# fegemo/palette-and-histo-gan

Hardware: AMD Instinct MI355X
Metric: train images/sec (64x64x4 sprites) (higher is better)
Workload: dtype bf16

## Files before the change

### palette_and_histo_gan_amd/csrc/conv_strip.hip

```cpp
#include "p2p_common.hpp"

struct CsArgs {
    const char* in; long long in_img; int in_row; int in_ld;
    char* out; long long out_img; int out_row; int out_ld;
    const char* w;
    float* stat_part;
    int LH, LW, lgLW;
    int TH, strips_per_img, nstrips;
    int RH, RW, PB;
    float inv_RW;
};

#define CS_MAXC 7
#define CS_THREADS 512

template <int MODE>
__global__ __launch_bounds__(CS_THREADS) void conv_strip_kernel(CsArgs a) {
    constexpr int NTAP = MODE == 1 ? 4 : 16;
    constexpr int KS = MODE == 1 ? 8 : 2;
    constexpr int CIN = KS * 16;
    constexpr int LGCPP = MODE == 1 ? 4 : 2;
    constexpr int PROW = 64 + 16;
    extern __shared__ __attribute__((aligned(16))) char smem[];
    const int tid = threadIdx.x, lane = tid & 63;
    const int wave = __builtin_amdgcn_readfirstlane(tid >> 6);
    const int h = lane >> 5, r = lane & 31;
    const int RW = a.RW, PB = a.PB;
    char* sL = smem;
    char* pL = smem + ((a.RH * RW * PB + 15) & ~15) + wave * (32 * PROW);
    const int slice = wave & 3, tpar = wave >> 2;
    const int ph = slice >> 1, pw = slice & 1;

    bf16x8 wf[NTAP][KS];
#pragma unroll
    for (int t = 0; t < NTAP; ++t) {
        int widx, row;
        if (MODE == 1) { widx = ((1 - ph) + 2 * (t >> 1)) * 4 + (1 - pw) + 2 * (t & 1); row = r; }
        else { widx = t; row = 32 * slice + r; }
        const int rows = MODE == 1 ? 32 : 128;
        const char* wp = a.w + ((long long)(widx * rows + row) * CIN) * 2;
#pragma unroll
        for (int ks = 0; ks < KS; ++ks) wf[t][ks] = *(const bf16x8*)(wp + (16 * ks + 8 * h) * 2);
    }

    const int nch = (a.RH * RW) << LGCPP;
    const int gpB = a.in_ld * 2;
    f32x4 stg[CS_MAXC];
    auto g_load = [&](int strip) {
        const int n = strip / a.strips_per_img, y0 = (strip - n * a.strips_per_img) * a.TH;
        const int oy = MODE == 1 ? y0 - 1 : 2 * y0 - 1;
        const char* base = a.in + ((long long)n * a.in_img + (long long)oy * a.in_row - 1) * gpB;
#pragma unroll
        for (int i = 0; i < CS_MAXC; ++i) {
            const int ci = tid + i * CS_THREADS;
            if (ci < nch) {
                const int px = ci >> LGCPP, cc = ci & ((1 << LGCPP) - 1);
                const int ry = (int)(((float)px + 0.5f) * a.inv_RW), rx = px - ry * RW;
                stg[i] = *(const f32x4*)(base + ((long long)ry * a.in_row + rx) * gpB + cc * 16);
            }
        }
    };
    auto l_store = [&]() {
#pragma unroll
        for (int i = 0; i < CS_MAXC; ++i) {
            const int ci = tid + i * CS_THREADS;
            if (ci < nch) *(f32x4*)(sL + (ci >> LGCPP) * PB + (ci & ((1 << LGCPP) - 1)) * 16) = stg[i];
        }
    };

    const int tiles = (a.TH * a.LW) >> 5;
    float* stL = (float*)(smem + ((a.RH * RW * PB + 15) & ~15) + 8 * (32 * PROW));
    int pend_n = -1, pend_s = 0;
    auto flush_stats = [&]() {
        if (tid < 32) {
            float s1 = 0.f, s2 = 0.f;
#pragma unroll
            for (int wv = 0; wv < 8; ++wv) { s1 += stL[(wv * 32 + tid) * 2]; s2 += stL[(wv * 32 + tid) * 2 + 1]; }
            const float cnt = (float)(4 * a.TH * a.LW);
            const float mean = s1 / cnt;
            float* dst = a.stat_part + (((long long)pend_n * a.strips_per_img + pend_s) * 32 + tid) * 2;
            dst[0] = mean;
            dst[1] = fmaxf(s2 - s1 * mean, 0.f);
        }
    };
    int strip = blockIdx.x;
    if (strip < a.nstrips) g_load(strip);
    for (; strip < a.nstrips; strip += gridDim.x) {
        __syncthreads();
        if (MODE == 1 && a.stat_part && pend_n >= 0) flush_stats();
        l_store();
        __syncthreads();
        if (strip + (int)gridDim.x < a.nstrips) g_load(strip + gridDim.x);
        const int n = strip / a.strips_per_img, sidx = strip - n * a.strips_per_img, y0 = sidx * a.TH;
        float ssum = 0.f, ssq = 0.f;
        for (int tile = tpar; tile < tiles; tile += 2) {
            const int p = tile * 32 + r;
            const int yy = p >> a.lgLW, x = p & (a.LW - 1);
            f32x16 acc;
            const float zero = p2p_valu_zero();
#pragma unroll
            for (int e = 0; e < 16; ++e) acc[e] = zero;
#pragma unroll
            for (int t = 0; t < NTAP; ++t) {
                int ry, rx;
                if (MODE == 1) {
                    const int kh = (1 - ph) + 2 * (t >> 1), kw = (1 - pw) + 2 * (t & 1);
                    ry = yy + 1 + ((ph + 1 - kh) >> 1);
                    rx = x + 1 + ((pw + 1 - kw) >> 1);
                } else { ry = 2 * yy + (t >> 2); rx = 2 * x + (t & 3); }
                const char* bp = sL + (ry * RW + rx) * PB + 16 * h;
#pragma unroll
                for (int ks = 0; ks < KS; ++ks) {
                    const bf16x8 b = *(const bf16x8*)(bp + 32 * ks);
                    acc = __builtin_amdgcn_mfma_f32_32x32x16_bf16(wf[t][ks], b, acc, 0, 0, 0);
                }
            }
#pragma unroll
            for (int g = 0; g < 4; ++g) {
                typedef __attribute__((__vector_size__(4 * sizeof(bf16_t)))) bf16_t bf16x4;
                bf16x4 q;
#pragma unroll
                for (int k = 0; k < 4; ++k) q[k] = (bf16_t)acc[4 * g + k];
                *(bf16x4*)(pL + r * PROW + (8 * g + 4 * h) * 2) = q;
            }
            asm volatile("s_waitcnt lgkmcnt(0)" ::: "memory");
            __builtin_amdgcn_wave_barrier();
            if (MODE == 1 && a.stat_part) {
                const bf16_t* col = (const bf16_t*)(pL + (16 * h) * PROW) + r;
#pragma unroll
                for (int i = 0; i < 16; ++i) {
                    const float v = (float)col[i * (PROW / 2)];
                    ssum += v;
                    ssq += v * v;
                }
            }
            const int ch = lane & 3, pq = lane >> 2;
#pragma unroll
            for (int ps = 0; ps < 32; ps += 16) {
                const int pix = ps + pq;
                const int pp = tile * 32 + pix;
                const int py = pp >> a.lgLW, px = pp & (a.LW - 1);
                const f32x4 v = *(const f32x4*)(pL + pix * PROW + ch * 16);
                long long opix;
                int c0;
                if (MODE == 1) { opix = (long long)n * a.out_img + (long long)(2 * (y0 + py) + ph) * a.out_row + (2 * px + pw); c0 = ch * 8; }
                else { opix = (long long)n * a.out_img + (long long)(y0 + py) * a.out_row + px; c0 = 32 * slice + ch * 8; }
                *(f32x4*)((bf16_t*)a.out + opix * a.out_ld + c0) = v;
            }
            __builtin_amdgcn_wave_barrier();
        }
        if (MODE == 1 && a.stat_part) {
            ssum += __shfl_xor(ssum, 32, 64);
            ssq += __shfl_xor(ssq, 32, 64);
            if (h == 0) { stL[(wave * 32 + r) * 2] = ssum; stL[(wave * 32 + r) * 2 + 1] = ssq; }
            pend_n = n; pend_s = sidx;
        }
    }
    if (MODE == 1 && a.stat_part && pend_n >= 0) {
        __syncthreads();
        flush_stats();
    }
}

struct CsPlan { int ok, TH, RH, RW, PB, blocks; size_t shm; };

static CsPlan cs_plan(int op, int dtype, int N, int LH, int LW, int Cg, int Cd) {
    CsPlan p = {0, 0, 0, 0, 0, 0, 0};
    if (dtype != P2P_BF16 || Cg != 32 || Cd != 128 || N < 1) return p;
    if (op != P2P_OP_G && op != P2P_OP_P) return p;
    if ((LW & (LW - 1)) || LW < 32 || LW > 128 || LH < 1) return p;
    const int cin = op == P2P_OP_P ? 128 : 32;
    p.PB = cin * 2 + 16;
    int TH = 0;
    for (int pass = 0; pass < 2 && !TH; ++pass)
        for (int t = 4; t >= (pass ? 1 : 2); t >>= 1) {
            if (t > LH || LH % t) continue;
            p.RH = op == P2P_OP_P ? t + 2 : 2 * t + 3;
            p.RW = op == P2P_OP_P ? LW + 2 : 2 * LW + 3;
            p.shm = (((size_t)p.RH * p.RW * p.PB + 15) & ~(size_t)15) + 8 * 32 * (size_t)(64 + 16) + 8 * 32 * 2 * sizeof(float);
            const long long nch = (long long)p.RH * p.RW * (cin / 8);
            if (nch > CS_MAXC * CS_THREADS) continue;
            if (((t * LW) >> 5) & 1) continue;
            if (p.shm <= (size_t)(pass ? 150 : 80) * 1024) { TH = t; break; }
        }
    if (!TH) return p;
    p.TH = TH;
    const long long strips = (long long)N * (LH / TH);
    if (strips > 0x7fffffffLL) return p;
    p.blocks = (int)(strips < 256 ? strips : 256);
    p.ok = 1;
    return p;
}

extern "C" int p2p_conv_strip_ok(int op, int dtype, int N, int LH, int LW, int Cg, int Cd) {
    return cs_plan(op, dtype, N, LH, LW, Cg, Cd).ok;
}

extern "C" int p2p_conv_strip_stat_slots(int op, int dtype, int N, int LH, int LW, int Cg, int Cd) {
    const CsPlan p = cs_plan(op, dtype, N, LH, LW, Cg, Cd);
    return (p.ok && op == P2P_OP_P) ? LH / p.TH : 0;
}

extern "C" int p2p_conv_strip(int op, int dtype, int N, int LH, int LW, int Cg, int Cd, const p2p_tensor* hi,
                              const p2p_tensor* lo, const void* w, float* stat_part, void* stream) {
    P2P_REQUIRE(hi && lo && hi->ptr && lo->ptr && w, "p2p_conv_strip: null pointer");
    const CsPlan p = cs_plan(op, dtype, N, LH, LW, Cg, Cd);
    P2P_REQUIRE(p.ok, "p2p_conv_strip: shape not supported (query p2p_conv_strip_ok)");
    const p2p_tensor* in = op == P2P_OP_G ? hi : lo;
    const p2p_tensor* out = op == P2P_OP_G ? lo : hi;
    const int cin = op == P2P_OP_P ? 128 : 32, cout = op == P2P_OP_P ? 32 : 128;
    P2P_REQUIRE(in->ld >= cin && in->ld % 8 == 0 && ((uintptr_t)in->ptr % 16) == 0 && ((uintptr_t)w % 16) == 0,
                "p2p_conv_strip: input view / weights must be 16-byte aligned");
    P2P_REQUIRE(out->ld >= cout && out->ld % 8 == 0 && ((uintptr_t)out->ptr % 16) == 0, "p2p_conv_strip: output view must be 16-byte aligned");
    CsArgs a;
    a.in = (const char*)in->ptr; a.in_img = in->img_stride; a.in_row = in->row_stride; a.in_ld = in->ld;
    a.out = (char*)out->ptr; a.out_img = out->img_stride; a.out_row = out->row_stride; a.out_ld = out->ld;
    a.w = (const char*)w;
    a.LH = LH; a.LW = LW;
    a.lgLW = 0;
    while ((1 << a.lgLW) < LW) ++a.lgLW;
    a.TH = p.TH; a.strips_per_img = LH / p.TH; a.nstrips = N * a.strips_per_img;
    a.RH = p.RH; a.RW = p.RW; a.PB = p.PB;
    a.inv_RW = 1.0f / (float)p.RW;
    a.stat_part = op == P2P_OP_P ? stat_part : nullptr;
    hipStream_t st = (hipStream_t)stream;
    const dim3 grid((unsigned)p.blocks);
    static bool attr_done = false;
    if (!attr_done)
        attr_done = (int)p2p_allow_lds((const void*)conv_strip_kernel<0>, 160 * 1024, "conv_strip_kernel<0>") &
                    (int)p2p_allow_lds((const void*)conv_strip_kernel<1>, 160 * 1024, "conv_strip_kernel<1>");
    if (op == P2P_OP_P) conv_strip_kernel<1><<<grid, dim3(CS_THREADS), p.shm, st>>>(a);
    else conv_strip_kernel<0><<<grid, dim3(CS_THREADS), p.shm, st>>>(a);
    return p2p_check_launch("p2p_conv_strip");
}
```

Baseline: 135,000.

## Carry halo rows between consecutive strips via LDS ring buffer

Switches from grid-strided strip assignment to contiguous strip ranges per block. Consecutive strips of the same image now reuse the two overlapping halo rows kept in an LDS ring buffer, so only the new rows are loaded from global memory. Tile x indexing is also simplified so each tile covers 32 pixels within one row. This adds ring-index arithmetic to the inner loop's address computation and relies on the assumption that a tile never straddles rows.

Result: no change. 136,300 (median of 6 runs) (+1.0%).

```diff
diff --git a/palette_and_histo_gan_amd/csrc/conv_strip.hip b/palette_and_histo_gan_amd/csrc/conv_strip.hip
--- a/palette_and_histo_gan_amd/csrc/conv_strip.hip
+++ b/palette_and_histo_gan_amd/csrc/conv_strip.hip
@@ -8,11 +8,16 @@
     int LH, LW, lgLW;
     int TH, strips_per_img, nstrips;
     int RH, RW, PB;
+    int RG;
     float inv_RW;
 };
 
 #define CS_MAXC 7
 #define CS_THREADS 512
+#define CS_KEEP 2
+#ifndef CS_CARRY_ROWS
+#define CS_CARRY_ROWS 1
+#endif
 
 template <int MODE>
 __global__ __launch_bounds__(CS_THREADS) void conv_strip_kernel(CsArgs a) {
@@ -25,7 +30,8 @@
     const int tid = threadIdx.x, lane = tid & 63;
     const int wave = __builtin_amdgcn_readfirstlane(tid >> 6);
     const int h = lane >> 5, r = lane & 31;
-    const int RW = a.RW, PB = a.PB;
+    const int RW = a.RW, PB = a.PB, RG = a.RG;
+    const int ring_px = RG * RW;
     char* sL = smem;
     char* pL = smem + ((a.RH * RW * PB + 15) & ~15) + wave * (32 * PROW);
     const int slice = wave & 3, tpar = wave >> 2;
@@ -43,12 +49,13 @@
         for (int ks = 0; ks < KS; ++ks) wf[t][ks] = *(const bf16x8*)(wp + (16 * ks + 8 * h) * 2);
     }
 
-    const int nch = (a.RH * RW) << LGCPP;
     const int gpB = a.in_ld * 2;
     f32x4 stg[CS_MAXC];
-    auto g_load = [&](int strip) {
+    auto g_load = [&](int strip, bool full) {
         const int n = strip / a.strips_per_img, y0 = (strip - n * a.strips_per_img) * a.TH;
-        const int oy = MODE == 1 ? y0 - 1 : 2 * y0 - 1;
+        const int j0 = full ? 0 : CS_KEEP;
+        const int oy = (MODE == 1 ? y0 - 1 : 2 * y0 - 1) + j0;
+        const int nch = ((RG - j0) * RW) << LGCPP;
         const char* base = a.in + ((long long)n * a.in_img + (long long)oy * a.in_row - 1) * gpB;
 #pragma unroll
         for (int i = 0; i < CS_MAXC; ++i) {
@@ -60,11 +67,20 @@
             }
         }
     };
-    auto l_store = [&]() {
+    auto l_store = [&](int rb, bool full) {
+        const int j0 = full ? 0 : CS_KEEP;
+        const int nch = ((RG - j0) * RW) << LGCPP;
+        int r0 = rb + j0;
+        if (r0 >= RG) r0 -= RG;
+        const int p0 = r0 * RW;
 #pragma unroll
         for (int i = 0; i < CS_MAXC; ++i) {
             const int ci = tid + i * CS_THREADS;
-            if (ci < nch) *(f32x4*)(sL + (ci >> LGCPP) * PB + (ci & ((1 << LGCPP) - 1)) * 16) = stg[i];
+            if (ci < nch) {
+                int px = p0 + (ci >> LGCPP);
+                if (px >= ring_px) px -= ring_px;
+                *(f32x4*)(sL + px * PB + (ci & ((1 << LGCPP) - 1)) * 16) = stg[i];
+            }
         }
     };
 
@@ -83,19 +99,25 @@
             dst[1] = fmaxf(s2 - s1 * mean, 0.f);
         }
     };
-    int strip = blockIdx.x;
-    if (strip < a.nstrips) g_load(strip);
-    for (; strip < a.nstrips; strip += gridDim.x) {
+    const int s_begin = (int)(((long long)blockIdx.x * a.nstrips) / (int)gridDim.x);
+    const int s_end = (int)(((long long)(blockIdx.x + 1) * a.nstrips) / (int)gridDim.x);
+    int rb = 0;
+    bool full = true;
+    if (s_begin < s_end) g_load(s_begin, true);
+    __builtin_amdgcn_s_waitcnt(0x0F70);
+    for (int strip = s_begin; strip < s_end; ++strip) {
+        const int n = strip / a.strips_per_img, sidx = strip - n * a.strips_per_img, y0 = sidx * a.TH;
         __syncthreads();
         if (MODE == 1 && a.stat_part && pend_n >= 0) flush_stats();
-        l_store();
+        l_store(rb, full);
         __syncthreads();
-        if (strip + (int)gridDim.x < a.nstrips) g_load(strip + gridDim.x);
-        const int n = strip / a.strips_per_img, sidx = strip - n * a.strips_per_img, y0 = sidx * a.TH;
+        const bool next_full = !CS_CARRY_ROWS || sidx + 1 == a.strips_per_img;
+        if (strip + 1 < s_end) g_load(strip + 1, next_full);
         float ssum = 0.f, ssq = 0.f;
-        for (int tile = tpar; tile < tiles; tile += 2) {
-            const int p = tile * 32 + r;
-            const int yy = p >> a.lgLW, x = p & (a.LW - 1);
+        int tile = tpar;
+        do {
+            const int yy = (tile * 32) >> a.lgLW;
+            const int x = ((tile * 32) & (a.LW - 1)) + r;
             f32x16 acc;
             const float zero = p2p_valu_zero();
 #pragma unroll
@@ -108,7 +130,9 @@
                     ry = yy + 1 + ((ph + 1 - kh) >> 1);
                     rx = x + 1 + ((pw + 1 - kw) >> 1);
                 } else { ry = 2 * yy + (t >> 2); rx = 2 * x + (t & 3); }
-                const char* bp = sL + (ry * RW + rx) * PB + 16 * h;
+                int rr = rb + ry;
+                if (rr >= RG) rr -= RG;
+                const char* bp = sL + (rr * RW + rx) * PB + 16 * h;
 #pragma unroll
                 for (int ks = 0; ks < KS; ++ks) {
                     const bf16x8 b = *(const bf16x8*)(bp + 32 * ks);
@@ -148,13 +172,17 @@
                 *(f32x4*)((bf16_t*)a.out + opix * a.out_ld + c0) = v;
             }
             __builtin_amdgcn_wave_barrier();
-        }
+            tile += 2;
+        } while (tile < tiles);
         if (MODE == 1 && a.stat_part) {
             ssum += __shfl_xor(ssum, 32, 64);
             ssq += __shfl_xor(ssq, 32, 64);
             if (h == 0) { stL[(wave * 32 + r) * 2] = ssum; stL[(wave * 32 + r) * 2 + 1] = ssq; }
             pend_n = n; pend_s = sidx;
         }
+        if (next_full) rb = 0;
+        else { rb += RG - CS_KEEP; if (rb >= RG) rb -= RG; }
+        full = next_full;
     }
     if (MODE == 1 && a.stat_part && pend_n >= 0) {
         __syncthreads();
@@ -221,6 +249,7 @@
     while ((1 << a.lgLW) < LW) ++a.lgLW;
     a.TH = p.TH; a.strips_per_img = LH / p.TH; a.nstrips = N * a.strips_per_img;
     a.RH = p.RH; a.RW = p.RW; a.PB = p.PB;
+    a.RG = op == P2P_OP_P ? p.TH + 2 : 2 * p.TH + 2;
     a.inv_RW = 1.0f / (float)p.RW;
     a.stat_part = op == P2P_OP_P ? stat_part : nullptr;
     hipStream_t st = (hipStream_t)stream;
```
